# dremovd/PPO

Hardware: AMD Instinct MI355X
Metric: env-steps/sec (Pong-shaped synthetic, 256 envs/GPU) (higher is better)
Workload: dtype f32

## Files before the change

### ppo_amd/csrc/stack_fused.hip

```cpp
#include <cstdlib>
#include <type_traits>

#include "common.h"
#include "conv_stage.h"
#include "mfma.h"

#ifndef PPO_TAIL_SPLIT
#define PPO_TAIL_SPLIT 2
#endif

namespace ppo {
namespace {

constexpr int kScrPitchS = 20;

struct StackTailArgs {
    const float *in;
    const float *w[4];
    const float *bias[4];
    const float *mask[4];
    float *save[4];
    int n_images;
};

// ... 149 lines not shown

            __builtin_amdgcn_sched_barrier(0);
            load_weights((layer + 1) & 3);
            float *dst = smem + (odd ? 0 : S::LDS_MAP);
            float *save = a.save[layer];
            __builtin_amdgcn_sched_barrier(0);
            float skip[MT][NT][4];
#pragma unroll
            for (int m = 0; m < MT; ++m)
#pragma unroll
                for (int n = 0; n < NT; ++n)
#pragma unroll
                    for (int r = 0; r < 4; ++r)
                        skip[m][n][r] = odd ? smem[((n0 + n) * 16 + g * 4 + r) * PLANE + G + W + (pix[m] < S::NPIX ? pix[m] : 0)] : 0.f;
#pragma unroll
            for (int m = 0; m < MT; ++m) {
                if (pix[m] < S::NPIX) {
#pragma unroll
                    for (int n = 0; n < NT; ++n)
#pragma unroll
                        for (int r = 0; r < 4; ++r) {
                            const int co = (n0 + n) * 16 + g * 4 + r;
                            const int lo = co * PLANE + G + W + pix[m];
                            float val = acc[n][m][r] + bias_r[n][r];
                            if constexpr (BACKWARD) val = gate[m][n][r] > 0.f ? val : 0.f;
                            if (odd) val = val + skip[m][n][r];
                            dst[lo] = val;
                            if (save) save[img_off + (size_t)co * (H * W) + pix[m]] = val;
                        }
                }
            }
        }
    }
}

template <int C, int H, int W, int MT, int NW, int NSPLIT, bool BACKWARD>
int launch_stack_tail(const StackTailArgs &args, hipStream_t st)
{
    using S = StackCfg<C, H, W, MT, NW, NSPLIT>;
    auto kern = stack_tail_kernel<C, H, W, MT, NW, NSPLIT, BACKWARD>;
    static int wg_per_cu = 0;
    if (wg_per_cu == 0) {
        hipError_t e = hipFuncSetAttribute(reinterpret_cast<const void *>(kern), hipFuncAttributeMaxDynamicSharedMemorySize,
                                           (int)S::LDS_BYTES);
        if (e != hipSuccess) return fail(PPO_E_HIP, "stack_tail: hipFuncSetAttribute: %s", hipGetErrorString(e));
        int nb = 0;
        e = hipOccupancyMaxActiveBlocksPerMultiprocessor(&nb, kern, S::WAVES * 64, S::LDS_BYTES);
        if (e != hipSuccess) return fail(PPO_E_HIP, "stack_tail: occupancy query: %s", hipGetErrorString(e));
        wg_per_cu = nb < 1 ? 1 : nb;
    }
    int grid = 256 * wg_per_cu;
    if (grid > args.n_images) grid = args.n_images;
    hipLaunchKernelGGL(kern, dim3(grid), dim3(S::WAVES * 64), S::LDS_BYTES, st, args);
    return check_launch("stack_tail_kernel");
}

template <int C, int H, int W, int TR>
struct ShiftCfg {
    static_assert(C == 16, "one channel tile per wave");
    static constexpr int NW = 16;
    static constexpr int GW = 8;
    static constexpr int G = 4;
    static constexpr int ROWS = H + 6;
    static constexpr int PLANE_RAW = ROWS * W + 2 * G;
    static constexpr int PLANE = PLANE_RAW + ((16 - PLANE_RAW % 32) + 32) % 32;
    static constexpr int KS = 9 * (C / 4);
    static constexpr int NBANDS = (H + TR - 1) / TR;
    static constexpr int NPIX = TR * W;
    static constexpr int MTILES = (NPIX + 15) / 16;
    static constexpr int MT = MTILES / GW;
    static constexpr int LDS_MAP = C * PLANE;
    static constexpr int SCR = MT * 16 * kScrPitchS;
    static constexpr size_t LDS_BYTES = (size_t)(LDS_MAP + GW * SCR) * 4;
    static_assert(H % TR == 0 && MTILES == MT * GW, "whole bands, tiles split evenly over a group's waves");
    static_assert((H * W) % 4 == 0 && NPIX % 4 == 0 && W % 2 == 0, "float4 epilogue on whole quads");
    static_assert(LDS_BYTES <= 160 * 1024, "map + scratch must fit the CU's LDS");
};

template <int C, int H, int W, int TR, bool BACKWARD>
__global__ __launch_bounds__(1024) void stack_shift_kernel(StackTailArgs a)
{
    using S = ShiftCfg<C, H, W, TR>;
    constexpr int KS = S::KS, PLANE = S::PLANE, G = S::G, MT = S::MT, NW = S::NW;
    extern __shared__ __align__(16) float smem[];
    const int tid = threadIdx.x, lane = tid & 63, l15 = lane & 15, g = lane >> 4, wave = tid >> 6;
    const int grp = __builtin_amdgcn_readfirstlane(wave / S::GW), wv = wave % S::GW;
    const int ch = lane >> 2, quad = lane & 3;
    float *scr = smem + S::LDS_MAP + wv * S::SCR;

    int lofs[MT], p4[MT];
    float hi_l[MT], hi_r[MT];
#pragma unroll
    for (int m = 0; m < MT; ++m) {
        const int p = (wv * MT + m) * 16 + l15;
        lofs[m] = G + p - 1 + g * PLANE;
        hi_l[m] = (p % W == 0) ? 0.f : INFINITY;
        hi_r[m] = (p % W == W - 1) ? 0.f : INFINITY;
        p4[m] = (wv * MT + m) * 16 + quad * 4;
    }

    for (int img = blockIdx.x; img < a.n_images; img += gridDim.x) {
        const size_t img_off = (size_t)img * C * H * W;
        __syncthreads();
        for (int i = tid; i < C * 6 * W; i += NW * 64) {
            const int c = i / (6 * W), r = (i / W) % 6, x = i % W;
            smem[c * PLANE + G + (r < 5 ? r : H + 5) * W + x] = 0.f;
        }
        for (int i = tid; i < C * 2 * G; i += NW * 64)
            smem[(i / (2 * G)) * PLANE + ((i % (2 * G)) < G ? (i % G) : G + S::ROWS * W + (i % G))] = 0.f;
        {
            using gptr_t = const __attribute__((address_space(1))) void *;
            using lptr_t = __attribute__((address_space(3))) void *;
            constexpr int N4 = H * W / 4, REQ = (N4 + 63) / 64;
            const int w0 = __builtin_amdgcn_readfirstlane(wave);
            for (int c = w0; c < C; c += NW) {
                const float *g0 = a.in + img_off + (size_t)c * H * W;
                float *l0 = smem + c * PLANE + G + 5 * W;
#pragma unroll
                for (int q = 0; q < REQ; ++q)
                    if (q * 64 + lane < N4)
                        __builtin_amdgcn_global_load_lds((gptr_t)(g0 + (q * 64 + lane) * 4), (lptr_t)(l0 + q * 256), 16, 0, 0);
            }
        }

#pragma unroll 1
        for (int layer = 0; layer < 4; ++layer) {
            float wa[KS];
            const float4 *pw = reinterpret_cast<const float4 *>(a.w[layer]);
#pragma unroll
            for (int s4 = 0; s4 < KS / 4; ++s4) {
                const float4 v = pw[s4 * 64 + lane];
                wa[4 * s4 + 0] = v.x, wa[4 * s4 + 1] = v.y, wa[4 * s4 + 2] = v.z, wa[4 * s4 + 3] = v.w;
            }
            const float bias_c = BACKWARD ? 0.f : a.bias[layer][ch];
            const int odd = layer & 1;
            const float *res = odd ? (layer == 1 ? a.in : a.save[1]) + img_off : nullptr;
            const float *mask = BACKWARD ? a.mask[layer] + img_off : nullptr;
            float *save = a.save[layer] ? a.save[layer] + img_off : nullptr;
            const __amdgpu_buffer_rsrc_t mask_b = buffer_of(mask, mask != nullptr), res_b = buffer_of(res, res != nullptr);
            const int in_row = 5 - layer;

            f32x4 acc[MT];
            float4 gate4[MT], res4[MT];

            __syncthreads();
#pragma unroll 1
            for (int hs = 0; hs <= S::NBANDS; ++hs) {
                if ((hs & 1) == grp) {
                    if (hs < S::NBANDS) {
                        const int y0 = hs * TR;
                        const int chan_off = ch * (H * W) + y0 * W;
#pragma unroll
                        for (int m = 0; m < MT; ++m) {
                            const bool live = p4[m] < S::NPIX;
                            const int off = live ? (chan_off + p4[m]) * 4 : kOutside;
                            if constexpr (BACKWARD) gate4[m] = buffer_f32x4(mask_b, off);
                            res4[m] = buffer_f32x4(res_b, off);
                        }
                        int base[MT];
#pragma unroll
                        for (int m = 0; m < MT; ++m) {
                            base[m] = lofs[m] + (y0 - 1 + in_row) * W;
                            acc[m] = f32x4{0.f, 0.f, 0.f, 0.f};
                        }
                        constexpr int SB = 2;
                        constexpr int NB = (KS + SB - 1) / SB;
                        float raw[2][SB][MT];
                        auto load_block = [&](int j, float (&r)[SB][MT]) {
#pragma unroll
                            for (int u = 0; u < SB; ++u) {
                                const int s = j * SB + u;
                                if (s < KS) {
                                    const int tap = s / (C / 4), cs = s % (C / 4);
                                    const int tap_off = (tap / 3) * W + (tap % 3);
#pragma unroll
                                    for (int m = 0; m < MT; ++m) r[u][m] = smem[base[m] + cs * 4 * PLANE + tap_off];
                                }
                            }
                        };
                        load_block(0, raw[0]);
#pragma unroll
                        for (int j = 0; j < NB; ++j) {
                            float bv[SB][MT];
#pragma unroll
                            for (int u = 0; u < SB; ++u) {
                                const int s = j * SB + u;
                                if (s < KS) {
                                    const int kx = (s / (C / 4)) % 3;
#pragma unroll
                                    for (int m = 0; m < MT; ++m) {
                                        float x = raw[j & 1][u][m];
                                        if (kx != 1) {
                                            const float hi = kx == 0 ? hi_l[m] : hi_r[m];
                                            x = __builtin_amdgcn_fmed3f(x, BACKWARD ? -hi : 0.f, hi);
                                        } else if (!BACKWARD) {
                                            x = relu1(x);
                                        }
                                        bv[u][m] = x;
                                    }
                                }
                            }
                            __builtin_amdgcn_sched_barrier(0);
                            if (j + 1 < NB) load_block(j + 1, raw[(j + 1) & 1]);
#pragma unroll
                            for (int u = 0; u < SB; ++u) {
                                const int s = j * SB + u;
                                if (s < KS) {
#pragma unroll
                                    for (int m = 0; m < MT; ++m) acc[m] = mfma16(wa[s], bv[u][m], acc[m]);
                                }
                            }
                            __builtin_amdgcn_sched_barrier(0);
                        }
                    } else if (layer < 3) {
                        for (int i = tid % (S::GW * 64); i < C * W; i += S::GW * 64)
                            smem[(i / W) * PLANE + G + (H + in_row - 1) * W + i % W] = 0.f;
                    }
                } else if (hs >= 1) {
                    const int y0 = (hs - 1) * TR;
                    const int chan_off = ch * (H * W) + y0 * W;
#pragma unroll
                    for (int m = 0; m < MT; ++m)
#pragma unroll
                        for (int r = 0; r < 4; ++r) scr[(m * 16 + g * 4 + r) * kScrPitchS + l15] = acc[m][r];
                    __builtin_amdgcn_wave_barrier();
                    float *out_row = smem + ch * PLANE + G + (y0 + in_row - 1) * W;
#pragma unroll
                    for (int m = 0; m < MT; ++m) {
                        if (p4[m] >= S::NPIX) continue;
                        const float4 o = *reinterpret_cast<const float4 *>(scr + (m * 16 + ch) * kScrPitchS + quad * 4);
                        const float ov[4] = {o.x, o.y, o.z, o.w};
                        const float gv[4] = {gate4[m].x, gate4[m].y, gate4[m].z, gate4[m].w};
                        const float rv[4] = {res4[m].x, res4[m].y, res4[m].z, res4[m].w};
                        float v[4];
#pragma unroll
                        for (int e = 0; e < 4; ++e) {
                            float val = ov[e] + bias_c;
                            if constexpr (BACKWARD) val = gv[e] > 0.f ? val : 0.f;
                            v[e] = val + rv[e];
                        }
                        if (layer < 3) {
                            *reinterpret_cast<float2 *>(out_row + p4[m]) = make_float2(v[0], v[1]);
                            *reinterpret_cast<float2 *>(out_row + p4[m] + 2) = make_float2(v[2], v[3]);
                        }
                        if (save) *reinterpret_cast<float4 *>(save + chan_off + p4[m]) = make_float4(v[0], v[1], v[2], v[3]);
                    }
                    __builtin_amdgcn_wave_barrier();
                }
                __syncthreads();
            }
        }
    }
}

template <int C, int H, int W, int TR, bool BACKWARD>
int launch_stack_shift(const StackTailArgs &args, hipStream_t st)
{
    using S = ShiftCfg<C, H, W, TR>;
    auto kern = stack_shift_kernel<C, H, W, TR, BACKWARD>;
    static bool attr_set = false;
    if (!attr_set) {
        hipError_t e = hipFuncSetAttribute(reinterpret_cast<const void *>(kern), hipFuncAttributeMaxDynamicSharedMemorySize,
                                           (int)S::LDS_BYTES);
        if (e != hipSuccess) return fail(PPO_E_HIP, "stack_shift: hipFuncSetAttribute: %s", hipGetErrorString(e));
        attr_set = true;
    }
    int grid = 256;
    if (grid > args.n_images) grid = args.n_images;
    hipLaunchKernelGGL(kern, dim3(grid), dim3(S::NW * 64), S::LDS_BYTES, st, args);
    return check_launch("stack_shift_kernel");
}

template <int I, int N, class F>
__device__ __forceinline__ void static_for(F &&f)
{
    if constexpr (I < N) {
        f(std::integral_constant<int, I>{});
        static_for<I + 1, N>(f);
    }
}

struct LaneMap {
    template <int MT>
    struct T {
        int pix[MT], lofs[MT];
        float hi_l[MT], hi_r[MT];
    };
};

template <int H, int W, int PLANE, int G, int MT>
__device__ __forceinline__ void lane_map_init(LaneMap::T<MT> &lm, int pixel_wave, int l15, int g)
{
#pragma unroll
    for (int m = 0; m < MT; ++m) {
        const int p = (pixel_wave * MT + m) * 16 + l15;
        lm.pix[m] = p;
        const int pc = p < H * W ? p : 0;
        lm.lofs[m] = G + pc - 1 + g * PLANE;
        lm.hi_l[m] = (pc % W == 0) ? 0.f : INFINITY;
        lm.hi_r[m] = (pc % W == W - 1) ? 0.f : INFINITY;
    }
}

template <int C, int H, int W, int MT, int NTOT, int NT, bool RELU_IN, bool GATED = false>
__device__ __forceinline__ void resident_conv(float *smem, int src_off, int dst_off, bool residual, const float *wpk,
                                              const float *bias, float *save, const LaneMap::T<MT> &lm, int n0, int lane,
                                              const float *mask = nullptr)
{
    constexpr int ROWS = H + 2, G = 4, PLANE_RAW = ROWS * W + 2 * G;
    constexpr int PLANE = PLANE_RAW + ((16 - PLANE_RAW % 32) + 32) % 32;
    constexpr int KS = 9 * (C / 4);
    const int g = lane >> 4;
    float wa[NT][KS];
    const float4 *pw = reinterpret_cast<const float4 *>(wpk);
#pragma unroll
    for (int s4 = 0; s4 < KS / 4; ++s4)
#pragma unroll
        for (int n = 0; n < NT; ++n) {
            const float4 v = pw[(s4 * NTOT + n0 + n) * 64 + lane];
            wa[n][4 * s4 + 0] = v.x;
            wa[n][4 * s4 + 1] = v.y;
            wa[n][4 * s4 + 2] = v.z;
            wa[n][4 * s4 + 3] = v.w;
        }
    float bias_r[NT][4];
#pragma unroll
    for (int n = 0; n < NT; ++n)
#pragma unroll
        for (int r = 0; r < 4; ++r) bias_r[n][r] = (GATED || !bias) ? 0.f : bias[(n0 + n) * 16 + g * 4 + r];
    constexpr int SB = (MT * NT >= 4) ? 2 : 4;
    constexpr int NB = (KS + SB - 1) / SB;
    constexpr int GATE_AT = (GATED && MT * NT * 4 > 16) ? NB / 2 : -1;
    float gate[GATED ? MT : 1][NT][4];
    auto load_gate = [&]() {
        const __amdgpu_buffer_rsrc_t mask_b = buffer_of(mask);
#pragma unroll
        for (int m = 0; m < MT; ++m)
#pragma unroll
            for (int n = 0; n < NT; ++n)
#pragma unroll
                for (int r = 0; r < 4; ++r)
                    gate[m][n][r] = buffer_f32(mask_b, lm.pix[m] < H * W ? (((n0 + n) * 16 + g * 4 + r) * (H * W) + lm.pix[m]) * 4
                                                                         : kOutside);
    };
    if constexpr (GATED && GATE_AT < 0) load_gate();

    __syncthreads();
    int base[MT];
#pragma unroll
    for (int m = 0; m < MT; ++m) base[m] = lm.lofs[m] + src_off;
    f32x4 acc[NT][MT];
#pragma unroll
    for (int n = 0; n < NT; ++n)
#pragma unroll
        for (int m = 0; m < MT; ++m) acc[n][m] = f32x4{0.f, 0.f, 0.f, 0.f};

    float raw[2][SB][MT];
    auto load_block = [&](int j, float (&r)[SB][MT]) {
#pragma unroll
        for (int u = 0; u < SB; ++u) {
            const int s = j * SB + u;
            if (s < KS) {
                const int tap = s / (C / 4), cs = s % (C / 4);
                const int tap_off = (tap / 3) * W + (tap % 3);
#pragma unroll
                for (int m = 0; m < MT; ++m) r[u][m] = smem[base[m] + cs * 4 * PLANE + tap_off];
            }
        }
    };
    load_block(0, raw[0]);
    static_for<0, NB>([&](auto jc) {
        constexpr int j = decltype(jc)::value;
        float bv[SB][MT];
#pragma unroll
        for (int u = 0; u < SB; ++u) {
            const int s = j * SB + u;
            if (s < KS) {
                const int kx = (s / (C / 4)) % 3;
#pragma unroll
                for (int m = 0; m < MT; ++m) {
                    float x = raw[j & 1][u][m];
                    if (kx != 1) {
                        const float hi = kx == 0 ? lm.hi_l[m] : lm.hi_r[m];
                        x = __builtin_amdgcn_fmed3f(x, RELU_IN ? 0.f : -hi, hi);
                    } else if (RELU_IN) {
                        x = relu1(x);
                    }
                    bv[u][m] = x;
                }
            }
        }
        __builtin_amdgcn_sched_barrier(0);
        if constexpr (j + 1 < NB) load_block(j + 1, raw[(j + 1) & 1]);
        if constexpr (j == GATE_AT) load_gate();
#pragma unroll
        for (int u = 0; u < SB; ++u) {
            const int s = j * SB + u;
            if (s < KS) {
#pragma unroll
                for (int m = 0; m < MT; ++m)
#pragma unroll
                    for (int n = 0; n < NT; ++n) acc[n][m] = mfma16(wa[n][s], bv[u][m], acc[n][m]);
            }
        }
        __builtin_amdgcn_sched_barrier(0);
    });
#pragma unroll
    for (int m = 0; m < MT; ++m) {
        if (lm.pix[m] < H * W) {
#pragma unroll
            for (int n = 0; n < NT; ++n)
#pragma unroll
                for (int r = 0; r < 4; ++r) {
                    const int co = (n0 + n) * 16 + g * 4 + r;
                    const int lo = dst_off + co * PLANE + G + W + lm.pix[m];
                    float val = acc[n][m][r] + bias_r[n][r];
                    if constexpr (GATED) val = gate[m][n][r] > 0.f ? val : 0.f;
                    if (residual) val = val + smem[lo];
                    smem[lo] = val;
                    if (save) save[(size_t)co * (H * W) + lm.pix[m]] = val;
                }
        }
    }
}

struct StackFullArgs {
    const float *in;
    const float *w[5];
    const float *bias[5];
    float *pooled;
    uint8_t *argmax;
    float *save[4];
    const float *pre_w[4];
    const float *pre_bias[4];
    float *pre_save[4];
    int has_pre;
    int n_images;
};

template <int C, int HI, int WI, int MTI, int HO, int WO, int MTO, int NW, int NSPLIT>
__global__ __launch_bounds__(NW * NSPLIT * 64) void stack_full_kernel(StackFullArgs a)
{
    using SI = StackCfg<C, HI, WI, MTI, NW, NSPLIT>;
    using SO = StackCfg<C, HO, WO, MTO, NW, NSPLIT>;
    static_assert(HO == (HI + 1) / 2 && WO == (WI + 1) / 2, "3x3 / stride 2 / pad 1 pooling");
    static_assert(2 * SO::LDS_MAP <= SI::LDS_MAP, "the small maps reuse the input map's LDS");
    constexpr int NT = SI::NTL, WAVES = SI::WAVES, THREADS = WAVES * 64;
    constexpr int A_OFF = 0, B_OFF = SI::LDS_MAP, X_OFF = 0, Y_OFF = SO::LDS_MAP;
    extern __shared__ __align__(16) float smem[];
    const int tid = threadIdx.x, lane = tid & 63, l15 = lane & 15, g = lane >> 4;
    const int wave = tid >> 6, pixel_wave = wave % NW, n0 = (wave / NW) * NT;

    LaneMap::T<MTI> lmi;
    LaneMap::T<MTO> lmo;
    lane_map_init<HI, WI, SI::PLANE, SI::G, MTI>(lmi, pixel_wave, l15, g);
    lane_map_init<HO, WO, SO::PLANE, SO::G, MTO>(lmo, pixel_wave, l15, g);

    if (a.has_pre) zero_lds<SI::LDS_MAP, THREADS>(smem + B_OFF, tid);

    for (int img = blockIdx.x; img < a.n_images; img += gridDim.x) {
        __syncthreads();
        zero_lds<SI::LDS_MAP, THREADS>(smem + A_OFF, tid);
        __syncthreads();
        stage_band_chunk_dma<C, HI, WI, SI::ROWS, SI::PLANE, SI::G, WAVES>(a.in, img, 0, smem + A_OFF, tid);
        if (a.has_pre) {
            const size_t big_img = (size_t)img * C * HI * WI;
#pragma unroll 1
            for (int layer = 0; layer < 4; ++layer) {
                const int odd = layer & 1;
                float *save = a.pre_save[layer] ? a.pre_save[layer] + big_img : nullptr;
                resident_conv<C, HI, WI, MTI, SI::NT, NT, true>(smem, odd ? B_OFF : A_OFF, odd ? A_OFF : B_OFF, odd != 0,
                                                                a.pre_w[layer], a.pre_bias[layer], save, lmi, n0, lane);
            }
        }
        resident_conv<C, HI, WI, MTI, SI::NT, NT, false>(smem, A_OFF, B_OFF, false, a.w[0], a.bias[0], nullptr, lmi, n0, lane);
        __syncthreads();
        zero_lds<2 * SO::LDS_MAP, THREADS>(smem + X_OFF, tid);
        __syncthreads();
        {
            constexpr int RPW = 64 / WO;
            const int sub = lane / WO, xo = lane % WO;
            const size_t out_img = (size_t)img * C * HO * WO;
            for (int u0 = wave * RPW; u0 < C * HO; u0 += WAVES * RPW) {
                const int u = u0 + sub;
                const int co = u / HO, yo = u % HO;
                if (sub < RPW && co < C) {
                    const float *src = smem + B_OFF + co * SI::PLANE + SI::G + WI + (2 * yo - 1) * WI + 2 * xo - 1;
                    float best;
                    int best_tap;
                    pool_window_lds<HI % 2 == 0, WI % 2 == 0>(src, WI, yo > 0, 2 * yo + 1 < HI, xo > 0, 2 * xo + 1 < WI, best, best_tap);
                    smem[X_OFF + co * SO::PLANE + SO::G + WO + yo * WO + xo] = best;
                    const size_t oi = out_img + ((size_t)co * HO + yo) * WO + xo;
                    if (a.pooled) a.pooled[oi] = best;
                    if (a.argmax) a.argmax[oi] = (uint8_t)best_tap;
                }
            }
        }
        const size_t out_img = (size_t)img * C * HO * WO;
#pragma unroll 1
        for (int layer = 0; layer < 4; ++layer) {
            const int odd = layer & 1;
            float *save = a.save[layer] ? a.save[layer] + out_img : nullptr;
            resident_conv<C, HO, WO, MTO, SO::NT, NT, true>(smem, odd ? Y_OFF : X_OFF, odd ? X_OFF : Y_OFF, odd != 0,
                                                            a.w[1 + layer], a.bias[1 + layer], save, lmo, n0, lane);
        }
    }
}

struct StackFullBwdArgs {
    const float *g;
    const float *w[5];
    const float *mask[4];
    const uint8_t *argmax;
    float *save[4];
    float *dc;
    float *g_prev;
    const float *post_w[4];
    const float *post_mask[4];
    float *post_save[4];
    int has_post;
    int n_images;
};

template <int C, int HI, int WI, int MTI, int HO, int WO, int MTO, int NW, int NSPLIT>
__global__ __launch_bounds__(NW * NSPLIT * 64) void stack_full_bwd_kernel(StackFullBwdArgs a)
{
    using SI = StackCfg<C, HI, WI, MTI, NW, NSPLIT>;
    using SO = StackCfg<C, HO, WO, MTO, NW, NSPLIT>;
    static_assert(2 * SO::LDS_MAP <= SI::LDS_MAP, "the small maps live inside the first big map's LDS");
    static_assert(C * HO * WO <= SO::LDS_MAP * 4, "the argmax bytes of an image fit the second small map");
    constexpr int NT = SI::NTL, WAVES = SI::WAVES, THREADS = WAVES * 64;
    constexpr int A_OFF = 0, B_OFF = SI::LDS_MAP, X_OFF = 0, Y_OFF = SO::LDS_MAP;
    extern __shared__ __align__(16) float smem[];
    const int tid = threadIdx.x, lane = tid & 63, l15 = lane & 15, g = lane >> 4;
    const int wave = tid >> 6, pixel_wave = wave % NW, n0 = (wave / NW) * NT;

    LaneMap::T<MTI> lmi;
    LaneMap::T<MTO> lmo;
    lane_map_init<HI, WI, SI::PLANE, SI::G, MTI>(lmi, pixel_wave, l15, g);
    lane_map_init<HO, WO, SO::PLANE, SO::G, MTO>(lmo, pixel_wave, l15, g);

    zero_lds<SI::LDS_MAP, THREADS>(smem + B_OFF, tid);

    for (int img = blockIdx.x; img < a.n_images; img += gridDim.x) {
        __syncthreads();
        zero_lds<2 * SO::LDS_MAP, THREADS>(smem + X_OFF, tid);
        __syncthreads();
        stage_band_chunk_dma<C, HO, WO, SO::ROWS, SO::PLANE, SO::G, WAVES>(a.g, img, 0, smem + X_OFF, tid);
        const size_t small_img = (size_t)img * C * HO * WO, big_img = (size_t)img * C * HI * WI;
        constexpr int AM_WORDS = C * HO * WO / 4, AM_PER = (AM_WORDS + THREADS - 1) / THREADS;
        static_assert(C * HO * WO % 4 == 0, "an image's argmax bytes are whole words (the entry points check the base)");
        uint32_t am_r[AM_PER];
#pragma unroll
        for (int k = 0; k < AM_PER; ++k) {
            const int i = tid + k * THREADS;
            am_r[k] = reinterpret_cast<const uint32_t *>(a.argmax + small_img)[i < AM_WORDS ? i : 0];
        }
#pragma unroll 1
        for (int layer = 0; layer < 4; ++layer) {
            const int odd = layer & 1;
            resident_conv<C, HO, WO, MTO, SO::NT, NT, false, true>(smem, odd ? Y_OFF : X_OFF, odd ? X_OFF : Y_OFF, odd != 0,
                                                                   a.w[layer], nullptr, a.save[layer] + small_img, lmo, n0,
                                                                   lane, a.mask[layer] + small_img);
        }
        __syncthreads();
        const uint8_t *am = reinterpret_cast<const uint8_t *>(smem + Y_OFF);
#pragma unroll
        for (int k = 0; k < AM_PER; ++k) {
            const int i = tid + k * THREADS;
            if (i < AM_WORDS) reinterpret_cast<uint32_t *>(smem + Y_OFF)[i] = am_r[k];
        }
        __syncthreads();
        {
            for (int e = tid; e < C * HI * WI; e += THREADS) {
                const int co = e / (HI * WI), r = e % (HI * WI);
                const int iy = r / WI, ix = r % WI;
                const int k = ix >> 1, oy0 = iy >> 1;
                const int ky0 = (iy & 1) ? 2 : 1;
                const bool has_oy1 = (iy & 1) && (oy0 + 1 < HO);
                const bool odd_x = ix & 1;
                const bool has_ox1 = odd_x && (k + 1 < WO);
                const int kx0 = odd_x ? 2 : 1;
                const float *gx = smem + X_OFF + co * SO::PLANE + SO::G + WO;
                const uint8_t *ac = am + co * (HO * WO);
                float sum = 0.f;
                {
                    const int i00 = oy0 * WO + k;
                    if (ac[i00] == ky0 * 3 + kx0) sum += gx[i00];
                    if (has_ox1 && ac[i00 + 1] == ky0 * 3 + 0) sum += gx[i00 + 1];
                }
                if (has_oy1) {
                    const int i10 = (oy0 + 1) * WO + k;
                    if (ac[i10] == kx0) sum += gx[i10];
                    if (has_ox1 && ac[i10 + 1] == 0) sum += gx[i10 + 1];
                }
                smem[B_OFF + co * SI::PLANE + SI::G + WI + r] = sum;
                a.dc[big_img + e] = sum;
            }
        }
        if (a.has_post) {
            __syncthreads();
            zero_lds<SI::LDS_MAP, THREADS>(smem + A_OFF, tid);
        }
        resident_conv<C, HI, WI, MTI, SI::NT, NT, false, false>(smem, B_OFF, A_OFF, false, a.w[4], nullptr,
                                                                a.g_prev + big_img, lmi, n0, lane);
        if (a.has_post) {
#pragma unroll 1
            for (int layer = 0; layer < 4; ++layer) {
                const int odd = layer & 1;
                resident_conv<C, HI, WI, MTI, SI::NT, NT, false, true>(smem, odd ? B_OFF : A_OFF, odd ? A_OFF : B_OFF, odd != 0,
                                                                       a.post_w[layer], nullptr, a.post_save[layer] + big_img,
                                                                       lmi, n0, lane, a.post_mask[layer] + big_img);
            }
        }
    }
}

template <int C, int HI, int WI, int MTI, int HO, int WO, int MTO, int NW, int NSPLIT>
int launch_stack_full_bwd(const StackFullBwdArgs &args, hipStream_t st)
{
    using SI = StackCfg<C, HI, WI, MTI, NW, NSPLIT>;
    constexpr size_t kLds = 2 * (size_t)SI::LDS_MAP * 4;
    auto kern = stack_full_bwd_kernel<C, HI, WI, MTI, HO, WO, MTO, NW, NSPLIT>;
    static bool ready = false;
    if (!ready) {
        hipError_t e = hipFuncSetAttribute(reinterpret_cast<const void *>(kern), hipFuncAttributeMaxDynamicSharedMemorySize,
                                           (int)kLds);
        if (e != hipSuccess) return fail(PPO_E_HIP, "stack_full_bwd: hipFuncSetAttribute: %s", hipGetErrorString(e));
        ready = true;
    }
    const int grid = args.n_images < 256 ? args.n_images : 256;
    hipLaunchKernelGGL(kern, dim3(grid), dim3(SI::WAVES * 64), kLds, st, args);
    return check_launch("stack_full_bwd_kernel");
}

template <int C, int HI, int WI, int MTI, int HO, int WO, int MTO, int NW, int NSPLIT>
int launch_stack_full(const StackFullArgs &args, hipStream_t st)
{
    using SI = StackCfg<C, HI, WI, MTI, NW, NSPLIT>;
    constexpr size_t kLds = 2 * (size_t)SI::LDS_MAP * 4;
    auto kern = stack_full_kernel<C, HI, WI, MTI, HO, WO, MTO, NW, NSPLIT>;
    static bool ready = false;
    if (!ready) {
        hipError_t e = hipFuncSetAttribute(reinterpret_cast<const void *>(kern), hipFuncAttributeMaxDynamicSharedMemorySize,
                                           (int)kLds);
        if (e != hipSuccess) return fail(PPO_E_HIP, "stack_full: hipFuncSetAttribute: %s", hipGetErrorString(e));
        ready = true;
    }
    const int grid = args.n_images < 256 ? args.n_images : 256;
    hipLaunchKernelGGL(kern, dim3(grid), dim3(SI::WAVES * 64), kLds, st, args);
    return check_launch("stack_full_kernel");
}


struct ChainSplitArgs {
    const float *in;
    const float *pre_w[4];
    const float *pre_bias[4];
    const float *w[5];
    const float *bias[5];
    float *out;
    float *xbuf;
    uint32_t *flags;
    uint32_t *ctl;
    int n_images;
    int skip;
};

constexpr int kSplitWaves = 8;
constexpr uint32_t kSpinLimit = 1u << 21;

template <int C, int HI, int WI, int HO, int WO>
__global__ __launch_bounds__(kSplitWaves * 64) void stack_chain_split_kernel(ChainSplitArgs a)
{
    static_assert(C == 32, "two channel tiles: one per workgroup of a pair");
    using SI = StackCfg<C, HI, WI, 7, 4, 2>;
    using SO = StackCfg<C, HO, WO, 2, 4, 2>;
    constexpr int MTI = 4, MTO = 2, WAVES = kSplitWaves, THREADS = WAVES * 64;
    static_assert(SI::MTILES <= MTI * WAVES && SO::MTILES == MTO * 4 && WAVES == 8, "every pixel tile has a wave");
    static_assert(2 * SO::LDS_MAP <= SI::LDS_MAP, "the small maps reuse the input map's LDS");
    constexpr int A_OFF = 0, B_OFF = SI::LDS_MAP, X_OFF = 0, Y_OFF = SO::LDS_MAP;
    extern __shared__ __align__(16) float smem[];
    const int tid = threadIdx.x, lane = tid & 63, l15 = lane & 15, g = lane >> 4;
    const int wave = tid >> 6;
    const int b = blockIdx.x;
    const int h = (b >> 3) & 1;
    const int pair0 = (b & 7) | ((b >> 4) << 3);
    const int n_pairs = (gridDim.x >> 4) << 3;

    LaneMap::T<MTI> lmi;
    LaneMap::T<MTO> lmo;
    lane_map_init<HI, WI, SI::PLANE, SI::G, MTI>(lmi, wave, l15, g);
    lane_map_init<HO, WO, SO::PLANE, SO::G, MTO>(lmo, wave & 3, l15, g);

    const uint32_t base = __hip_atomic_load(a.ctl, __ATOMIC_RELAXED, __HIP_MEMORY_SCOPE_AGENT) * 8u;
    const uint32_t fault = __hip_atomic_load(a.ctl + 3, __ATOMIC_RELAXED, __HIP_MEMORY_SCOPE_AGENT);
    const uint32_t spin_limit = fault ? 1u << 10 : kSpinLimit;
    bool gave_up = false;
    zero_lds<SI::LDS_MAP, THREADS>(smem + B_OFF, tid);

    for (int img = pair0; img < a.n_images; img += n_pairs) {
        uint32_t *flag_own = a.flags + 2 * img + h, *flag_other = a.flags + 2 * img + (1 - h);
        float *slots = a.xbuf + (size_t)img * 2 * C * HI * WI;
        uint32_t step = 0;
        auto exchange = [&](int dst_off, float *slot, bool fetch) {
            ++step;
            asm volatile("s_waitcnt vmcnt(0)" ::: "memory");
            __syncthreads();
            if (tid == 0) {
                if (!(fault && h == 1))
                    __hip_atomic_store(flag_own, base + step, __ATOMIC_RELAXED, __HIP_MEMORY_SCOPE_AGENT);
                uint32_t it = 0;
                while (!(a.skip & 1) && !gave_up &&
                       __hip_atomic_load(flag_other, __ATOMIC_RELAXED, __HIP_MEMORY_SCOPE_AGENT) < base + step) {
                    if (++it > spin_limit ||
                        ((it & 1023u) == 0 && __hip_atomic_load(a.ctl + 2, __ATOMIC_RELAXED, __HIP_MEMORY_SCOPE_AGENT))) {
                        __hip_atomic_store(a.ctl + 2, 1u, __ATOMIC_RELAXED, __HIP_MEMORY_SCOPE_AGENT);
                        gave_up = true;
                        break;
                    }
                    __builtin_amdgcn_s_sleep(2);
                }
            }
            __syncthreads();
            if (fetch)
                stage_band_chunk_dma<16, HI, WI, SI::ROWS, SI::PLANE, SI::G, WAVES, 16>(slot + (size_t)(1 - h) * 16 * HI * WI, 0, 0,
                                                                                       smem + dst_off + (1 - h) * 16 * SI::PLANE, tid);
        };

        __syncthreads();
        zero_lds<SI::LDS_MAP, THREADS>(smem + A_OFF, tid);
        __syncthreads();
        stage_band_chunk_dma<C, HI, WI, SI::ROWS, SI::PLANE, SI::G, WAVES>(a.in, img, 0, smem + A_OFF, tid);
#pragma unroll 1
        for (int layer = 0; layer < 4; ++layer) {
            const int odd = layer & 1;
            float *slot = slots + (size_t)(layer & 1) * C * HI * WI;
            resident_conv<C, HI, WI, MTI, 2, 1, true>(smem, odd ? B_OFF : A_OFF, odd ? A_OFF : B_OFF, odd != 0, a.pre_w[layer],
                                                      a.pre_bias[layer], slot, lmi, h, lane);
            exchange(odd ? A_OFF : B_OFF, slot, true);
        }
        resident_conv<C, HI, WI, MTI, 2, 1, false>(smem, A_OFF, B_OFF, false, a.w[0], a.bias[0], slots, lmi, h, lane);
        exchange(B_OFF, slots, h == 0);
        if (h != 0 || (a.skip & 2)) continue;
        __syncthreads();
        zero_lds<2 * SO::LDS_MAP, THREADS>(smem + X_OFF, tid);
        __syncthreads();
        {
            constexpr int RPW = 64 / WO;
            const int sub = lane / WO, xo = lane % WO;
            for (int u0 = wave * RPW; u0 < C * HO; u0 += WAVES * RPW) {
                const int u = u0 + sub;
                const int co = u / HO, yo = u % HO;
                if (sub < RPW && co < C) {
                    const float *src = smem + B_OFF + co * SI::PLANE + SI::G + WI + (2 * yo - 1) * WI + 2 * xo - 1;
                    float best;
                    int best_tap;
                    pool_window_lds<HI % 2 == 0, WI % 2 == 0>(src, WI, yo > 0, 2 * yo + 1 < HI, xo > 0, 2 * xo + 1 < WI, best, best_tap);
                    smem[X_OFF + co * SO::PLANE + SO::G + WO + yo * WO + xo] = best;
                }
            }
        }
        float *out_img = a.out + (size_t)img * C * HO * WO;
#pragma unroll 1
        for (int layer = 0; layer < 4; ++layer) {
            const int odd = layer & 1;
            resident_conv<C, HO, WO, MTO, 2, 1, true>(smem, odd ? Y_OFF : X_OFF, odd ? X_OFF : Y_OFF, odd != 0, a.w[1 + layer],
                                                      a.bias[1 + layer], layer == 3 ? out_img : nullptr, lmo, wave >> 2, lane);
        }
    }
    __syncthreads();
    if (tid == 0) {
        const uint32_t done = __hip_atomic_fetch_add(a.ctl + 1, 1u, __ATOMIC_RELAXED, __HIP_MEMORY_SCOPE_AGENT);
        if (done == gridDim.x - 1) {
            __hip_atomic_store(a.ctl + 1, 0u, __ATOMIC_RELAXED, __HIP_MEMORY_SCOPE_AGENT);
            __hip_atomic_fetch_add(a.ctl, 1u, __ATOMIC_RELAXED, __HIP_MEMORY_SCOPE_AGENT);
        }
    }
}

template <int C, int HI, int WI, int HO, int WO>
int launch_chain_split(const ChainSplitArgs &args, hipStream_t st)
{
    using SI = StackCfg<C, HI, WI, 7, 4, 2>;
    constexpr size_t kLds = 2 * (size_t)SI::LDS_MAP * 4;
    auto kern = stack_chain_split_kernel<C, HI, WI, HO, WO>;
    static bool ready = false;
    if (!ready) {
        hipError_t e = hipFuncSetAttribute(reinterpret_cast<const void *>(kern), hipFuncAttributeMaxDynamicSharedMemorySize,
                                           (int)kLds);
        if (e != hipSuccess) return fail(PPO_E_HIP, "stack_chain_split: hipFuncSetAttribute: %s", hipGetErrorString(e));
        ready = true;
    }
    int groups = (args.n_images + 7) / 8;
    if (groups > 16) groups = 16;
    hipLaunchKernelGGL(kern, dim3(16 * groups), dim3(kSplitWaves * 64), kLds, st, args);
    return check_launch("stack_chain_split_kernel");
}

}
}

extern "C" int ppo_impala_stack_tail_supported(int channels, int h, int w)
{
    if (channels == 16) return (h == 42 && w == 42) || (h == 32 && w == 32);
    return channels == 32 && ((h == 11 && w == 11) || (h == 21 && w == 21) || (h == 16 && w == 16) || (h == 8 && w == 8));
}

extern "C" int ppo_impala_stack_tail_forward_f32(const float *in, const float *const *packed_weights,
                                                 const float *const *biases, float *a0, float *q0, float *a1, float *q1,
                                                 int n_images, int channels, int h, int w, void *stream)
{
    using namespace ppo;
    if (n_images < 0) return fail(PPO_E_INVALID, "ppo_impala_stack_tail_forward_f32: negative batch");
    if (n_images == 0) return PPO_OK;
    if (!in || !packed_weights || !biases || !q1)
        return fail(PPO_E_INVALID, "ppo_impala_stack_tail_forward_f32: null pointer");
    StackTailArgs args;
    args.in = in;
    for (int l = 0; l < 4; ++l) {
        if (!packed_weights[l] || !biases[l])
            return fail(PPO_E_INVALID, "ppo_impala_stack_tail_forward_f32: null weights / bias of layer %d", l);
        if (!aligned(packed_weights[l], 16))
            return fail(PPO_E_ALIGN, "ppo_impala_stack_tail_forward_f32: packed weights must be 16-byte aligned");
        args.w[l] = packed_weights[l];
        args.bias[l] = biases[l];
        args.mask[l] = nullptr;
    }
    if (!aligned(in, 4)) return fail(PPO_E_ALIGN, "ppo_impala_stack_tail_forward_f32: input must be 4-byte aligned");
    args.save[0] = a0;
    args.save[1] = q0;
    args.save[2] = a1;
    args.save[3] = q1;
    args.n_images = n_images;
    hipStream_t st = as_stream(stream);
    if (channels == 16) {
        if (!q0) return fail(PPO_E_INVALID, "ppo_impala_stack_tail_forward_f32: the 16-channel form needs q0 (its second block re-reads it)");
        if (!aligned(in, 16) || !aligned(q0, 16) || !aligned(q1, 16) || (a0 && !aligned(a0, 16)) || (a1 && !aligned(a1, 16)))
            return fail(PPO_E_ALIGN, "ppo_impala_stack_tail_forward_f32: the 16-channel form needs 16-byte aligned maps");
        if (h == 42 && w == 42) return launch_stack_shift<16, 42, 42, 6, false>(args, st);
        if (h == 32 && w == 32) return launch_stack_shift<16, 32, 32, 8, false>(args, st);
    }
    if (channels == 32 && h == 11 && w == 11) return launch_stack_tail<32, 11, 11, 2, 4, PPO_TAIL_SPLIT, false>(args, st);
    if (channels == 32 && h == 21 && w == 21) return launch_stack_tail<32, 21, 21, 7, 4, PPO_TAIL_SPLIT, false>(args, st);
    if (channels == 32 && h == 16 && w == 16) return launch_stack_tail<32, 16, 16, 4, 4, PPO_TAIL_SPLIT, false>(args, st);
    if (channels == 32 && h == 8 && w == 8) return launch_stack_tail<32, 8, 8, 1, 4, PPO_TAIL_SPLIT, false>(args, st);
    return fail(PPO_E_INVALID, "ppo_impala_stack_tail_forward_f32: no kernel for %d channels at %dx%d", channels, h, w);
}

extern "C" int ppo_impala_stack_tail_backward_f32(const float *g, const float *const *packed_weights_t,
                                                  const float *const *masks, float *da1, float *g1, float *da0, float *g0,
                                                  int n_images, int channels, int h, int w, void *stream)
{
    using namespace ppo;
    if (n_images < 0) return fail(PPO_E_INVALID, "ppo_impala_stack_tail_backward_f32: negative batch");
    if (n_images == 0) return PPO_OK;
    if (!g || !packed_weights_t || !masks || !da1 || !g1 || !da0 || !g0)
        return fail(PPO_E_INVALID, "ppo_impala_stack_tail_backward_f32: null pointer");
    StackTailArgs args;
    args.in = g;
    for (int l = 0; l < 4; ++l) {
        if (!packed_weights_t[l] || !masks[l])
            return fail(PPO_E_INVALID, "ppo_impala_stack_tail_backward_f32: null weights / mask of layer %d", l);
        if (!aligned(packed_weights_t[l], 16))
            return fail(PPO_E_ALIGN, "ppo_impala_stack_tail_backward_f32: packed weights must be 16-byte aligned");
        args.w[l] = packed_weights_t[l];
        args.bias[l] = nullptr;
        args.mask[l] = masks[l];
    }
    args.save[0] = da1;
    args.save[1] = g1;
    args.save[2] = da0;
    args.save[3] = g0;
    args.n_images = n_images;
    hipStream_t st = as_stream(stream);
    if (channels == 16) {
        for (const void *ptr : {(const void *)g, (const void *)da1, (const void *)g1, (const void *)da0, (const void *)g0,
                                (const void *)masks[0], (const void *)masks[1], (const void *)masks[2], (const void *)masks[3]})
            if (!aligned(ptr, 16))
                return fail(PPO_E_ALIGN, "ppo_impala_stack_tail_backward_f32: the 16-channel form needs 16-byte aligned maps");
        if (h == 42 && w == 42) return launch_stack_shift<16, 42, 42, 6, true>(args, st);
        if (h == 32 && w == 32) return launch_stack_shift<16, 32, 32, 8, true>(args, st);
    }
    if (channels == 32 && h == 11 && w == 11) return launch_stack_tail<32, 11, 11, 2, 4, PPO_TAIL_SPLIT, true>(args, st);
    if (channels == 32 && h == 21 && w == 21) return launch_stack_tail<32, 21, 21, 7, 4, PPO_TAIL_SPLIT, true>(args, st);
    if (channels == 32 && h == 16 && w == 16) return launch_stack_tail<32, 16, 16, 4, 4, PPO_TAIL_SPLIT, true>(args, st);
    if (channels == 32 && h == 8 && w == 8) return launch_stack_tail<32, 8, 8, 1, 4, PPO_TAIL_SPLIT, true>(args, st);
    return fail(PPO_E_INVALID, "ppo_impala_stack_tail_backward_f32: no kernel for %d channels at %dx%d", channels, h, w);
}

extern "C" int ppo_impala_stack_full_supported(int channels, int h, int w)
{
    return channels == 32 && ((h == 21 && w == 21) || (h == 16 && w == 16));
}

extern "C" int ppo_impala_stack_full_forward_f32(const float *in, const float *const *packed_weights,
                                                 const float *const *biases, float *pooled, uint8_t *argmax, float *a0,
                                                 float *q0, float *a1, float *q1, int n_images, int channels, int h, int w,
                                                 void *stream)
{
    using namespace ppo;
    if (n_images < 0) return fail(PPO_E_INVALID, "ppo_impala_stack_full_forward_f32: negative batch");
    if (n_images == 0) return PPO_OK;
    if (!in || !packed_weights || !biases || !q1)
        return fail(PPO_E_INVALID, "ppo_impala_stack_full_forward_f32: null pointer");
    StackFullArgs args;
    args.in = in;
    for (int l = 0; l < 5; ++l) {
        if (!packed_weights[l] || !biases[l])
            return fail(PPO_E_INVALID, "ppo_impala_stack_full_forward_f32: null weights / bias of layer %d", l);
        if (!aligned(packed_weights[l], 16))
            return fail(PPO_E_ALIGN, "ppo_impala_stack_full_forward_f32: packed weights must be 16-byte aligned");
        args.w[l] = packed_weights[l];
        args.bias[l] = biases[l];
    }
    args.pooled = pooled;
    args.argmax = argmax;
    args.save[0] = a0;
    args.save[1] = q0;
    args.save[2] = a1;
    args.save[3] = q1;
    args.has_pre = 0;
    for (int l = 0; l < 4; ++l) {
        args.pre_w[l] = nullptr;
        args.pre_bias[l] = nullptr;
        args.pre_save[l] = nullptr;
    }
    args.n_images = n_images;
    if (channels == 32 && h == 21 && w == 21)
        return launch_stack_full<32, 21, 21, 7, 11, 11, 2, 4, 2>(args, as_stream(stream));
    if (channels == 32 && h == 16 && w == 16)
        return launch_stack_full<32, 16, 16, 4, 8, 8, 1, 4, 2>(args, as_stream(stream));
    return fail(PPO_E_INVALID, "ppo_impala_stack_full_forward_f32: no kernel for %d channels at %dx%d", channels, h, w);
}

extern "C" int ppo_impala_stack_chain_forward_f32(const float *in, const float *const *pre_packed_weights,
                                                  const float *const *pre_biases, float *pre_a0, float *pre_q0,
                                                  float *pre_a1, float *pre_q1, const float *const *packed_weights,
                                                  const float *const *biases, float *pooled, uint8_t *argmax, float *a0,
                                                  float *q0, float *a1, float *q1, int n_images, int channels, int h, int w,
                                                  void *stream)
{
    using namespace ppo;
    if (n_images < 0) return fail(PPO_E_INVALID, "ppo_impala_stack_chain_forward_f32: negative batch");
    if (n_images == 0) return PPO_OK;
    if (!in || !pre_packed_weights || !pre_biases || !packed_weights || !biases || !q1)
        return fail(PPO_E_INVALID, "ppo_impala_stack_chain_forward_f32: null pointer");
    StackFullArgs args;
    args.in = in;
    for (int l = 0; l < 5; ++l) {
        if (!packed_weights[l] || !biases[l] || (l < 4 && (!pre_packed_weights[l] || !pre_biases[l])))
            return fail(PPO_E_INVALID, "ppo_impala_stack_chain_forward_f32: null weights / bias of layer %d", l);
        if (!aligned(packed_weights[l], 16) || (l < 4 && !aligned(pre_packed_weights[l], 16)))
            return fail(PPO_E_ALIGN, "ppo_impala_stack_chain_forward_f32: packed weights must be 16-byte aligned");
        args.w[l] = packed_weights[l];
        args.bias[l] = biases[l];
        if (l < 4) {
            args.pre_w[l] = pre_packed_weights[l];
            args.pre_bias[l] = pre_biases[l];
        }
    }
    args.pre_save[0] = pre_a0;
    args.pre_save[1] = pre_q0;
    args.pre_save[2] = pre_a1;
    args.pre_save[3] = pre_q1;
    args.has_pre = 1;
    args.pooled = pooled;
    args.argmax = argmax;
    args.save[0] = a0;
    args.save[1] = q0;
    args.save[2] = a1;
    args.save[3] = q1;
    args.n_images = n_images;
    if (channels == 32 && h == 21 && w == 21)
        return launch_stack_full<32, 21, 21, 7, 11, 11, 2, 4, 2>(args, as_stream(stream));
    if (channels == 32 && h == 16 && w == 16)
        return launch_stack_full<32, 16, 16, 4, 8, 8, 1, 4, 2>(args, as_stream(stream));
    return fail(PPO_E_INVALID, "ppo_impala_stack_chain_forward_f32: no kernel for %d channels at %dx%d", channels, h, w);
}

extern "C" int ppo_impala_stack_full_backward_f32(const float *g, const float *const *packed_weights_t,
                                                  const float *const *masks, const uint8_t *argmax, float *da1, float *g1,
                                                  float *da0, float *g0, float *dc, float *g_prev, int n_images,
                                                  int channels, int h, int w, void *stream)
{
    using namespace ppo;
    if (n_images < 0) return fail(PPO_E_INVALID, "ppo_impala_stack_full_backward_f32: negative batch");
    if (n_images == 0) return PPO_OK;
    if (!g || !packed_weights_t || !masks || !argmax || !da1 || !g1 || !da0 || !g0 || !dc || !g_prev)
        return fail(PPO_E_INVALID, "ppo_impala_stack_full_backward_f32: null pointer");
    if (!aligned(argmax, 4)) return fail(PPO_E_ALIGN, "ppo_impala_stack_full_backward_f32: argmax must be 4-byte aligned");
    StackFullBwdArgs args;
    args.g = g;
    for (int l = 0; l < 5; ++l) {
        if (!packed_weights_t[l] || (l < 4 && !masks[l]))
            return fail(PPO_E_INVALID, "ppo_impala_stack_full_backward_f32: null weights / mask of layer %d", l);
        if (!aligned(packed_weights_t[l], 16))
            return fail(PPO_E_ALIGN, "ppo_impala_stack_full_backward_f32: packed weights must be 16-byte aligned");
        args.w[l] = packed_weights_t[l];
        if (l < 4) args.mask[l] = masks[l];
    }
    args.argmax = argmax;
    args.save[0] = da1;
    args.save[1] = g1;
    args.save[2] = da0;
    args.save[3] = g0;
    args.dc = dc;
    args.g_prev = g_prev;
    for (int l = 0; l < 4; ++l) {
        args.post_w[l] = nullptr;
        args.post_mask[l] = nullptr;
        args.post_save[l] = nullptr;
    }
    args.has_post = 0;
    args.n_images = n_images;
    if (channels == 32 && h == 21 && w == 21)
        return launch_stack_full_bwd<32, 21, 21, 7, 11, 11, 2, 4, 2>(args, as_stream(stream));
    if (channels == 32 && h == 16 && w == 16)
        return launch_stack_full_bwd<32, 16, 16, 4, 8, 8, 1, 4, 2>(args, as_stream(stream));
    return fail(PPO_E_INVALID, "ppo_impala_stack_full_backward_f32: no kernel for %d channels at %dx%d", channels, h, w);
}

extern "C" int ppo_impala_stack_chain_backward_f32(const float *g, const float *const *packed_weights_t,
                                                   const float *const *masks, const uint8_t *argmax, float *da1, float *g1,
                                                   float *da0, float *g0, float *dc, float *g_prev,
                                                   const float *const *post_packed_weights_t, const float *const *post_masks,
                                                   float *post_da1, float *post_g1, float *post_da0, float *post_g0,
                                                   int n_images, int channels, int h, int w, void *stream)
{
    using namespace ppo;
    if (n_images < 0) return fail(PPO_E_INVALID, "ppo_impala_stack_chain_backward_f32: negative batch");
    if (n_images == 0) return PPO_OK;
    if (!g || !packed_weights_t || !masks || !argmax || !da1 || !g1 || !da0 || !g0 || !dc || !g_prev || !post_packed_weights_t
        || !post_masks || !post_da1 || !post_g1 || !post_da0 || !post_g0)
        return fail(PPO_E_INVALID, "ppo_impala_stack_chain_backward_f32: null pointer");
    if (!aligned(argmax, 4)) return fail(PPO_E_ALIGN, "ppo_impala_stack_chain_backward_f32: argmax must be 4-byte aligned");
    StackFullBwdArgs args;
    args.g = g;
    for (int l = 0; l < 5; ++l) {
        if (!packed_weights_t[l] || (l < 4 && (!masks[l] || !post_packed_weights_t[l] || !post_masks[l])))
            return fail(PPO_E_INVALID, "ppo_impala_stack_chain_backward_f32: null weights / mask of layer %d", l);
        if (!aligned(packed_weights_t[l], 16) || (l < 4 && !aligned(post_packed_weights_t[l], 16)))
            return fail(PPO_E_ALIGN, "ppo_impala_stack_chain_backward_f32: packed weights must be 16-byte aligned");
        args.w[l] = packed_weights_t[l];
        if (l < 4) {
            args.mask[l] = masks[l];
            args.post_w[l] = post_packed_weights_t[l];
            args.post_mask[l] = post_masks[l];
        }
    }
    args.argmax = argmax;
    args.save[0] = da1;
    args.save[1] = g1;
    args.save[2] = da0;
    args.save[3] = g0;
    args.dc = dc;
    args.g_prev = g_prev;
    args.post_save[0] = post_da1;
    args.post_save[1] = post_g1;
    args.post_save[2] = post_da0;
    args.post_save[3] = post_g0;
    args.has_post = 1;
    args.n_images = n_images;
    if (channels == 32 && h == 21 && w == 21)
        return launch_stack_full_bwd<32, 21, 21, 7, 11, 11, 2, 4, 2>(args, as_stream(stream));
    if (channels == 32 && h == 16 && w == 16)
        return launch_stack_full_bwd<32, 16, 16, 4, 8, 8, 1, 4, 2>(args, as_stream(stream));
    return fail(PPO_E_INVALID, "ppo_impala_stack_chain_backward_f32: no kernel for %d channels at %dx%d", channels, h, w);
}

extern "C" size_t ppo_impala_stack_chain_split_workspace_bytes(int n_images, int channels, int h, int w)
// ... 51 lines not shown
```

Measured before the change: 98610.

## Prefetch next layer's packed conv weights into registers during current layer epilogue

Weight registers are now owned by the caller. Each resident_conv loads the next layer's packed A-operand right after its MFMA loop and before the epilogue stores, so the global weight fetch overlaps the store phase instead of stalling the start of the next layer. The chain is threaded across the layers in every kernel, including the wrap to the next image. Residual reads from LDS are also moved ahead of the store loop. This adds register pressure and some complex next-pointer and n0 selection logic, which could lower occupancy or cause spills.

```diff
diff --git a/ppo_amd/csrc/stack_fused.hip b/ppo_amd/csrc/stack_fused.hip
--- a/ppo_amd/csrc/stack_fused.hip
+++ b/ppo_amd/csrc/stack_fused.hip
@@ -475,16 +475,9 @@
     }
 }
 
-template <int C, int H, int W, int MT, int NTOT, int NT, bool RELU_IN, bool GATED = false>
-__device__ __forceinline__ void resident_conv(float *smem, int src_off, int dst_off, bool residual, const float *wpk,
-                                              const float *bias, float *save, const LaneMap::T<MT> &lm, int n0, int lane,
-                                              const float *mask = nullptr)
-{
-    constexpr int ROWS = H + 2, G = 4, PLANE_RAW = ROWS * W + 2 * G;
-    constexpr int PLANE = PLANE_RAW + ((16 - PLANE_RAW % 32) + 32) % 32;
-    constexpr int KS = 9 * (C / 4);
-    const int g = lane >> 4;
-    float wa[NT][KS];
+template <int NTOT, int NT, int KS>
+__device__ __forceinline__ void load_packed_a(float (&wa)[NT][KS], const float *wpk, int n0, int lane)
+{
     const float4 *pw = reinterpret_cast<const float4 *>(wpk);
 #pragma unroll
     for (int s4 = 0; s4 < KS / 4; ++s4)
@@ -496,6 +489,18 @@
             wa[n][4 * s4 + 2] = v.z;
             wa[n][4 * s4 + 3] = v.w;
         }
+}
+
+template <int C, int H, int W, int MT, int NTOT, int NT, bool RELU_IN, bool GATED = false>
+__device__ __forceinline__ void resident_conv(float *smem, int src_off, int dst_off, bool residual,
+                                              float (&wa)[NT][9 * (C / 4)], const float *next_w, int next_n0,
+                                              const float *bias, float *save, const LaneMap::T<MT> &lm, int n0, int lane,
+                                              const float *mask = nullptr)
+{
+    constexpr int ROWS = H + 2, G = 4, PLANE_RAW = ROWS * W + 2 * G;
+    constexpr int PLANE = PLANE_RAW + ((16 - PLANE_RAW % 32) + 32) % 32;
+    constexpr int KS = 9 * (C / 4);
+    const int g = lane >> 4;
     float bias_r[NT][4];
 #pragma unroll
     for (int n = 0; n < NT; ++n)
@@ -578,6 +583,18 @@
         }
         __builtin_amdgcn_sched_barrier(0);
     });
+    __builtin_amdgcn_sched_barrier(0);
+    if (next_w) load_packed_a<NTOT, NT, KS>(wa, next_w, next_n0, lane);
+    __builtin_amdgcn_sched_barrier(0);
+    float skip[MT][NT][4];
+#pragma unroll
+    for (int m = 0; m < MT; ++m)
+#pragma unroll
+        for (int n = 0; n < NT; ++n)
+#pragma unroll
+            for (int r = 0; r < 4; ++r)
+                skip[m][n][r] = residual ? smem[dst_off + ((n0 + n) * 16 + g * 4 + r) * PLANE + G + W + (lm.pix[m] < H * W ? lm.pix[m] : 0)]
+                                         : 0.f;
 #pragma unroll
     for (int m = 0; m < MT; ++m) {
         if (lm.pix[m] < H * W) {
@@ -589,7 +606,7 @@
                     const int lo = dst_off + co * PLANE + G + W + lm.pix[m];
                     float val = acc[n][m][r] + bias_r[n][r];
                     if constexpr (GATED) val = gate[m][n][r] > 0.f ? val : 0.f;
-                    if (residual) val = val + smem[lo];
+                    if (residual) val = val + skip[m][n][r];
                     smem[lo] = val;
                     if (save) save[(size_t)co * (H * W) + lm.pix[m]] = val;
                 }
@@ -629,6 +646,10 @@
     lane_map_init<HI, WI, SI::PLANE, SI::G, MTI>(lmi, pixel_wave, l15, g);
     lane_map_init<HO, WO, SO::PLANE, SO::G, MTO>(lmo, pixel_wave, l15, g);
 
+    const float *first_w = a.has_pre ? a.pre_w[0] : a.w[0];
+    float wa[NT][SI::KS];
+    load_packed_a<SI::NT, NT, SI::KS>(wa, first_w, n0, lane);
+
     if (a.has_pre) zero_lds<SI::LDS_MAP, THREADS>(smem + B_OFF, tid);
 
     for (int img = blockIdx.x; img < a.n_images; img += gridDim.x) {
@@ -642,11 +663,13 @@
             for (int layer = 0; layer < 4; ++layer) {
                 const int odd = layer & 1;
                 float *save = a.pre_save[layer] ? a.pre_save[layer] + big_img : nullptr;
-                resident_conv<C, HI, WI, MTI, SI::NT, NT, true>(smem, odd ? B_OFF : A_OFF, odd ? A_OFF : B_OFF, odd != 0,
-                                                                a.pre_w[layer], a.pre_bias[layer], save, lmi, n0, lane);
-            }
-        }
-        resident_conv<C, HI, WI, MTI, SI::NT, NT, false>(smem, A_OFF, B_OFF, false, a.w[0], a.bias[0], nullptr, lmi, n0, lane);
+                const float *next_w = layer < 3 ? a.pre_w[layer + 1] : a.w[0];
+                resident_conv<C, HI, WI, MTI, SI::NT, NT, true>(smem, odd ? B_OFF : A_OFF, odd ? A_OFF : B_OFF, odd != 0, wa,
+                                                                next_w, n0, a.pre_bias[layer], save, lmi, n0, lane);
+            }
+        }
+        resident_conv<C, HI, WI, MTI, SI::NT, NT, false>(smem, A_OFF, B_OFF, false, wa, a.w[1], n0, a.bias[0], nullptr, lmi, n0,
+                                                         lane);
         __syncthreads();
         zero_lds<2 * SO::LDS_MAP, THREADS>(smem + X_OFF, tid);
         __syncthreads();
@@ -670,12 +693,14 @@
             }
         }
         const size_t out_img = (size_t)img * C * HO * WO;
+        const bool more = img + (int)gridDim.x < a.n_images;
 #pragma unroll 1
         for (int layer = 0; layer < 4; ++layer) {
             const int odd = layer & 1;
             float *save = a.save[layer] ? a.save[layer] + out_img : nullptr;
-            resident_conv<C, HO, WO, MTO, SO::NT, NT, true>(smem, odd ? Y_OFF : X_OFF, odd ? X_OFF : Y_OFF, odd != 0,
-                                                            a.w[1 + layer], a.bias[1 + layer], save, lmo, n0, lane);
+            const float *next_w = layer < 3 ? a.w[2 + layer] : (more ? first_w : nullptr);
+            resident_conv<C, HO, WO, MTO, SO::NT, NT, true>(smem, odd ? Y_OFF : X_OFF, odd ? X_OFF : Y_OFF, odd != 0, wa, next_w,
+                                                            n0, a.bias[1 + layer], save, lmo, n0, lane);
         }
     }
 }
@@ -713,9 +738,13 @@
     lane_map_init<HI, WI, SI::PLANE, SI::G, MTI>(lmi, pixel_wave, l15, g);
     lane_map_init<HO, WO, SO::PLANE, SO::G, MTO>(lmo, pixel_wave, l15, g);
 
+    float wa[NT][SI::KS];
+    load_packed_a<SI::NT, NT, SI::KS>(wa, a.w[0], n0, lane);
+
     zero_lds<SI::LDS_MAP, THREADS>(smem + B_OFF, tid);
 
     for (int img = blockIdx.x; img < a.n_images; img += gridDim.x) {
+        const bool more = img + (int)gridDim.x < a.n_images;
         __syncthreads();
         zero_lds<2 * SO::LDS_MAP, THREADS>(smem + X_OFF, tid);
         __syncthreads();
@@ -732,9 +761,9 @@
 #pragma unroll 1
         for (int layer = 0; layer < 4; ++layer) {
             const int odd = layer & 1;
-            resident_conv<C, HO, WO, MTO, SO::NT, NT, false, true>(smem, odd ? Y_OFF : X_OFF, odd ? X_OFF : Y_OFF, odd != 0,
-                                                                   a.w[layer], nullptr, a.save[layer] + small_img, lmo, n0,
-                                                                   lane, a.mask[layer] + small_img);
+            resident_conv<C, HO, WO, MTO, SO::NT, NT, false, true>(smem, odd ? Y_OFF : X_OFF, odd ? X_OFF : Y_OFF, odd != 0, wa,
+                                                                   a.w[layer + 1], n0, nullptr, a.save[layer] + small_img, lmo,
+                                                                   n0, lane, a.mask[layer] + small_img);
         }
         __syncthreads();
         const uint8_t *am = reinterpret_cast<const uint8_t *>(smem + Y_OFF);
@@ -775,15 +804,17 @@
             __syncthreads();
             zero_lds<SI::LDS_MAP, THREADS>(smem + A_OFF, tid);
         }
-        resident_conv<C, HI, WI, MTI, SI::NT, NT, false, false>(smem, B_OFF, A_OFF, false, a.w[4], nullptr,
-                                                                a.g_prev + big_img, lmi, n0, lane);
+        resident_conv<C, HI, WI, MTI, SI::NT, NT, false, false>(smem, B_OFF, A_OFF, false, wa,
+                                                                a.has_post ? a.post_w[0] : (more ? a.w[0] : nullptr), n0,
+                                                                nullptr, a.g_prev + big_img, lmi, n0, lane);
         if (a.has_post) {
 #pragma unroll 1
             for (int layer = 0; layer < 4; ++layer) {
                 const int odd = layer & 1;
-                resident_conv<C, HI, WI, MTI, SI::NT, NT, false, true>(smem, odd ? B_OFF : A_OFF, odd ? A_OFF : B_OFF, odd != 0,
-                                                                       a.post_w[layer], nullptr, a.post_save[layer] + big_img,
-                                                                       lmi, n0, lane, a.post_mask[layer] + big_img);
+                const float *next_w = layer < 3 ? a.post_w[layer + 1] : (more ? a.w[0] : nullptr);
+                resident_conv<C, HI, WI, MTI, SI::NT, NT, false, true>(smem, odd ? B_OFF : A_OFF, odd ? A_OFF : B_OFF, odd != 0, wa,
+                                                                       next_w, n0, nullptr, a.post_save[layer] + big_img, lmi,
+                                                                       n0, lane, a.post_mask[layer] + big_img);
             }
         }
     }
@@ -872,7 +903,12 @@
     bool gave_up = false;
     zero_lds<SI::LDS_MAP, THREADS>(smem + B_OFF, tid);
 
+    const bool small_part = h == 0 && !(a.skip & 2);
+    float wa[1][SI::KS];
+    if (pair0 < a.n_images) load_packed_a<2, 1, SI::KS>(wa, a.pre_w[0], h, lane);
+
     for (int img = pair0; img < a.n_images; img += n_pairs) {
+        const bool more = img + n_pairs < a.n_images;
         uint32_t *flag_own = a.flags + 2 * img + h, *flag_other = a.flags + 2 * img + (1 - h);
         float *slots = a.xbuf + (size_t)img * 2 * C * HI * WI;
         uint32_t step = 0;
@@ -909,13 +945,16 @@
         for (int layer = 0; layer < 4; ++layer) {
             const int odd = layer & 1;
             float *slot = slots + (size_t)(layer & 1) * C * HI * WI;
-            resident_conv<C, HI, WI, MTI, 2, 1, true>(smem, odd ? B_OFF : A_OFF, odd ? A_OFF : B_OFF, odd != 0, a.pre_w[layer],
+            const float *next_w = layer < 3 ? a.pre_w[layer + 1] : a.w[0];
+            resident_conv<C, HI, WI, MTI, 2, 1, true>(smem, odd ? B_OFF : A_OFF, odd ? A_OFF : B_OFF, odd != 0, wa, next_w, h,
                                                       a.pre_bias[layer], slot, lmi, h, lane);
             exchange(odd ? A_OFF : B_OFF, slot, true);
         }
-        resident_conv<C, HI, WI, MTI, 2, 1, false>(smem, A_OFF, B_OFF, false, a.w[0], a.bias[0], slots, lmi, h, lane);
+        resident_conv<C, HI, WI, MTI, 2, 1, false>(smem, A_OFF, B_OFF, false, wa,
+                                                   small_part ? a.w[1] : (more ? a.pre_w[0] : nullptr), small_part ? wave >> 2 : h,
+                                                   a.bias[0], slots, lmi, h, lane);
         exchange(B_OFF, slots, h == 0);
-        if (h != 0 || (a.skip & 2)) continue;
+        if (!small_part) continue;
         __syncthreads();
         zero_lds<2 * SO::LDS_MAP, THREADS>(smem + X_OFF, tid);
         __syncthreads();
@@ -938,8 +977,10 @@
 #pragma unroll 1
         for (int layer = 0; layer < 4; ++layer) {
             const int odd = layer & 1;
-            resident_conv<C, HO, WO, MTO, 2, 1, true>(smem, odd ? Y_OFF : X_OFF, odd ? X_OFF : Y_OFF, odd != 0, a.w[1 + layer],
-                                                      a.bias[1 + layer], layer == 3 ? out_img : nullptr, lmo, wave >> 2, lane);
+            const float *next_w = layer < 3 ? a.w[2 + layer] : (more ? a.pre_w[0] : nullptr);
+            resident_conv<C, HO, WO, MTO, 2, 1, true>(smem, odd ? Y_OFF : X_OFF, odd ? X_OFF : Y_OFF, odd != 0, wa, next_w,
+                                                      layer < 3 ? wave >> 2 : h, a.bias[1 + layer],
+                                                      layer == 3 ? out_img : nullptr, lmo, wave >> 2, lane);
         }
     }
     __syncthreads();
```

Measured after the change: 99460 (median of 5 runs). Within noise of the previous version (+0.9%).
